# superlinear-ai/raglite

Measured on AMD Instinct MI355X. Metric: queries/sec, MaxSim 32x1M d=1024 exact top-100, higher is better.
Workload: dtype f32 in / f32 scores: candidate chunks found with the fp16 hi halves of corpus and queries (1 x v_mfma_f32_16x16x32_f16 per multiply, f32 accumulate, rigorous error bound), their scores by v_mfma_f32_16x16x4_f32 (exact f32 products); full-precision fallback: 3 x v_mfma_f32_16x16x32_f16 on hi+lo pairs

## Files before the change

### include/raglite_hip.h

```cpp
#ifndef RAGLITE_HIP_H
#define RAGLITE_HIP_H

#include <stddef.h>
#include <stdint.h>

#ifdef __cplusplus
extern "C" {
#endif

typedef enum {
    RL_OK = 0,
    RL_ERR_INVALID = -1,
    RL_ERR_HIP = -2,
    RL_ERR_UNSUPPORTED = -3,
    RL_ERR_NOMEM = -4
} rl_status;

typedef enum { RL_MEM_HOST = 0, RL_MEM_DEVICE = 1 } rl_mem;
typedef enum {
    RL_ARITH_AUTO = 0,
    RL_ARITH_FP32_EXACT = 1,
    RL_ARITH_F16_SPLIT = 2,
    RL_ARITH_F16_STORED = 3
} rl_arith;
// ... 44 lines not shown
int rl_index_delete_chunks(rl_index* index, const int64_t* chunk_ordinals, int64_t n, void* stream);
int rl_index_live(rl_index* index, int64_t* live_rows, int64_t* live_chunks, void* stream);
int rl_index_compact(rl_index* index, int64_t* out_remap, int64_t* new_n_rows, int64_t* new_n_chunks, void* stream);

int rl_index_set_arithmetic(rl_index* index, int mode);
int rl_index_arithmetic(rl_index* index, int* in_effect);

typedef enum {
    RL_OPT_HI_SEARCH = 1, RL_OPT_HI_MAXSIM = 2, RL_OPT_HI_PRODUCTS = 3, RL_OPT_PP_PASS = 4, RL_OPT_FUSED_TOPK = 5, RL_OPT_FUSED_HI = 6,
    RL_OPT_FUSED_PP = 7, RL_OPT_FUSED_TOPK_CAP = 8, RL_OPT_FUSED_TOPK_STRIDE = 9, RL_OPT_GEMM_PASS = 10, RL_OPT_QUERY_PAIRS = 11,
    RL_OPT_PLANES_GEMM = 12, RL_OPT_KEEP_IMAGE = 13, RL_OPT_KEEP_HI = 14, RL_OPT_IMAGE_HEADROOM_MB = 15, RL_OPT_ARITHMETIC = 16,
    RL_OPT_EXACT_KTH_THRESHOLD = 17, RL_OPT_FUSED_TWO_ROUNDS = 18, RL_OPT_KEEP_HI_PLANE = 19, RL_OPT_PAIRS_PACKED = 20,
    RL_OPT_F16_EXACT = 21, RL_OPT_LAZY_IMAGES = 22, RL_OPT_FUSED_PP_SAMPLE = 23,
    RL_OPT_LIST_SELECT = 24, RL_OPT_HI_FEW = 25, RL_OPT_TOPK_BLOCK = 26, RL_OPT_HI_PIVOT = 27, RL_OPT_COUNT_ = 28
} rl_option;
int rl_set_default_option(int key, int64_t value);
int rl_get_default_option(int key, int64_t* value);
int rl_index_set_option(rl_index* index, int key, int64_t value);
int rl_index_get_option(rl_index* index, int key, int64_t* value);

int rl_search_rows(rl_index* index, const float* queries, int32_t n_queries, int32_t k,
                   float* out_scores, int32_t* out_rows, int mem, void* stream);

int rl_rank_cut_begin(rl_index* index, const float* queries, int32_t n_queries, int mem, void* stream);
int rl_rank_cut_level(rl_index* index, int level, int64_t rank_limit, uint32_t* out_hist, int mem, void* stream);
int rl_rank_cut_level_done(rl_index* index, int level, const uint32_t* hist_sum, int mem, void* stream);
int rl_rank_cut_ties(rl_index* index, int64_t rank_limit, uint32_t* out_ties, int mem, void* stream);
int rl_rank_cut_finish(rl_index* index, int64_t rank_limit, const uint32_t* ties_before, const uint32_t* chunk_filter, int32_t k,
                       float* out_scores, int32_t* out_rows, int mem, void* stream);

// ... 90 lines not shown
```

### raglite_amd/_abi.py

```python

from __future__ import annotations

import ctypes as C
import functools
import os
from pathlib import Path

LIB_PATH = Path(os.environ.get("RAGLITE_HIP_LIB") or Path(__file__).resolve().parent / "_lib" / "libraglite_hip.so")

RL_OK, RL_ERR_INVALID, RL_ERR_HIP, RL_ERR_UNSUPPORTED, RL_ERR_NOMEM = 0, -1, -2, -3, -4
MEM_HOST, MEM_DEVICE = 0, 1
METRICS = {"cosine": 0, "dot": 1, "l2": 2}
SYNTH_KINDS = {"uniform": 0, "small_int": 1}
OPTIONS = {
    "hi_search": 1, "hi_maxsim": 2, "hi_products": 3, "pp_pass": 4, "fused_topk": 5, "fused_hi": 6, "fused_pp": 7, "fused_topk_cap": 8,
    "fused_topk_stride": 9, "gemm_pass": 10, "query_pairs": 11, "planes_gemm": 12, "keep_image": 13, "keep_hi": 14,
    "image_headroom_mb": 15, "arithmetic": 16, "exact_kth_threshold": 17, "fused_two_rounds": 18,
    "keep_hi_plane": 19, "pairs_packed": 20, "f16_exact": 21, "lazy_images": 22, "fused_pp_sample": 23, "list_select": 24, "hi_few": 25, "topk_block": 26, "hi_pivot": 27,
}

c_void_p, c_int, c_i32, c_i64, c_u64, c_size_t = C.c_void_p, C.c_int, C.c_int32, C.c_int64, C.c_uint64, C.c_size_t
c_double, c_char_p = C.c_double, C.c_char_p

_SIGNATURES = {
    "rl_version": [],
    "rl_last_error": [],
    "rl_init": [c_int],
    "rl_device_count": [C.POINTER(c_int)],
    "rl_device_info": [c_int, c_char_p, c_int, C.POINTER(c_int), C.POINTER(c_i64)],
    "rl_dev_alloc": [C.POINTER(c_void_p), c_size_t],
    "rl_dev_free": [c_void_p],
    "rl_memcpy_h2d": [c_void_p, c_void_p, c_size_t, c_void_p],
    "rl_memcpy_d2h": [c_void_p, c_void_p, c_size_t, c_void_p],
    "rl_memcpy_d2d": [c_void_p, c_void_p, c_size_t, c_void_p],
# ... 135 lines not shown
```

### raglite_amd/_build.py

```python

from __future__ import annotations

import os
import subprocess
import sys
from concurrent.futures import ThreadPoolExecutor
from pathlib import Path

PKG = Path(__file__).resolve().parent
CSRC = PKG / "csrc"
INCLUDE = PKG.parent / "include"
LIB_DIR = PKG / "_lib"
LIB_PATH = LIB_DIR / "libraglite_hip.so"
SOURCES = ["api.hip", "synth.hip", "pool_norm.hip", "scan.hip", "select.hip", "maxsim_stream.hip", "maxsim_generic.hip",
           "maxsim_gemm.hip", "maxsim_pp.hip", "score_gemm.hip", "mask.hip", "scan16.hip", "adapter_fit.hip", "partition_sim.hip", "comm.hip", "hi_filter.hip",
           "keyword.hip"]
FLAGS = ["--offload-arch=gfx950", "-O3", "-std=c++17", "-fPIC", "-Wall", "-Wno-unused-function",
         f"-I{INCLUDE}", f"-I{CSRC}"]


def _hipcc() -> str:
    for cand in (os.environ.get("HIPCC"), "/opt/rocm/bin/hipcc", "hipcc"):
        if cand and (os.path.isabs(cand) and os.path.exists(cand) or not os.path.isabs(cand)):
            return cand
# ... 4 lines not shown
    if not target.exists():
        return True
    t = target.stat().st_mtime
    return any(d.stat().st_mtime > t for d in deps)


EXP_LIB_PATH = LIB_DIR / "libraglite_hip_exp.so"


def build(force: bool = False, verbose: bool = False, experiments: bool = False) -> Path:
    LIB_DIR.mkdir(exist_ok=True)
    obj_dir = LIB_DIR / ("obj_exp" if experiments else "obj")
    obj_dir.mkdir(exist_ok=True)
    lib_path = EXP_LIB_PATH if experiments else LIB_PATH
    flags = FLAGS + (["-DRAGLITE_EXPERIMENTS"] if experiments else [])
    headers = [CSRC / "common.h", INCLUDE / "raglite_hip.h"]
    hipcc = _hipcc()

    def compile_one(src: str) -> Path:
        obj = obj_dir / (src + ".o")
        if force or _newer(obj, [CSRC / src, *headers]):
            cmd = [hipcc, *flags, "-c", str(CSRC / src), "-o", str(obj)]
            if verbose:
                print(" ".join(cmd), file=sys.stderr)
            res = subprocess.run(cmd, capture_output=True, text=True)
            if res.returncode != 0:
                raise RuntimeError(f"hipcc failed for {src}:\n{res.stderr}")
        return obj

    with ThreadPoolExecutor(max_workers=min(8, os.cpu_count() or 1)) as pool:
        objs = list(pool.map(compile_one, SOURCES))
# ... 11 lines not shown
```

### raglite_amd/_ops.py

```python

from __future__ import annotations

import ctypes as C
import threading
from typing import Any

import numpy as np

from raglite_amd import _abi
from raglite_amd._abi import MEM_DEVICE, MEM_HOST, METRICS, SYNTH_KINDS, check, lib

K_MAX = 2048


def _is_torch(x: Any) -> bool:
    return type(x).__module__.split(".")[0] == "torch"


def _torch():
    import torch

    return torch


# ... 59 lines not shown


def _ensure_init(device: int) -> None:
    if getattr(_tls, "initialised", None) != device:
        _abi.init(device)
        _tls.initialised = device
        _tls.device = device


def set_device(device: int) -> None:
    _tls.device = device
    _ensure_init(device)


def set_default_option(name: str, value: int) -> None:
    check(lib().rl_set_default_option(_abi.OPTIONS[name], int(value)))


def get_default_option(name: str) -> int:
    v = C.c_int64(0)
    check(lib().rl_get_default_option(_abi.OPTIONS[name], C.byref(v)))
    return int(v.value)


def synth_fill(out, seed: int, start: int = 0, kind: str = "uniform"):
    a = _Args()
    ptr = a.inp(out, np.float32)
    if a.mem != MEM_DEVICE or a.keep[0].data_ptr() != out.data_ptr():
        raise ValueError("synth_fill needs a contiguous float32 CUDA tensor")
    a.ensure_device()
    check(lib().rl_synth_fill(ptr, start, out.numel(), seed, SYNTH_KINDS[kind], a.stream))
    return out


def pool_norm(tokens, span_begin, span_end, *, normalize: bool = True, eps: float = 0.0,
              want_f32: bool = False, want_f16: bool = True):
# ... 189 lines not shown

    def compact(self) -> np.ndarray:
        _ensure_init(self.device.index or 0) if self.mem == MEM_DEVICE else _ensure_init(_current_device())
        remap = np.empty(self.n_chunks, dtype=np.int64)
        n_rows, n_chunks = C.c_int64(0), C.c_int64(0)
        check(lib().rl_index_compact(self._handle, remap.ctypes.data, C.byref(n_rows), C.byref(n_chunks), None))
        if int(n_chunks.value) != self.n_chunks:
            if self.chunk_offsets is not None:
                sizes = np.diff(self.chunk_offsets)[remap >= 0]
                self.chunk_offsets = np.concatenate(([0], np.cumsum(sizes))).astype(np.int64)
            self.n_rows, self.n_chunks = int(n_rows.value), int(n_chunks.value)
            self._keep = None
        return remap

    def set_option(self, name: str, value: int) -> None:
        check(lib().rl_index_set_option(self._handle, _abi.OPTIONS[name], int(value)))

    def get_option(self, name: str) -> int:
        v = C.c_int64(0)
        check(lib().rl_index_get_option(self._handle, _abi.OPTIONS[name], C.byref(v)))
        return int(v.value)

    def options(self, **kv: int):
        index = self

        class _Ctx:
            def __enter__(self):
                self.old = {k: index.get_option(k) for k in kv}
                for k, v in kv.items():
                    index.set_option(k, v)
                return index

            def __exit__(self, *exc):
                for k, v in self.old.items():
                    index.set_option(k, v)
# ... 287 lines not shown
```

### raglite_amd/csrc/api.hip

```cpp
#include <cmath>
#include <cstdlib>
#include <cstring>
#include <limits>
#include <memory>
#include <mutex>
#include <utility>
#include <vector>

#include "common.h"

namespace rl {

static thread_local std::string g_last_error;
void set_error(const std::string& msg) { g_last_error = msg; }
int fail(int code, const std::string& msg) {
    g_last_error = msg;
    return code;
}

namespace {

hipStream_t as_stream(void* s) { return reinterpret_cast<hipStream_t>(s); }

struct BlockCache {
// ... 165 lines not shown
    return RL_OK;
}

int scan_mode(int metric) {
    switch (metric) {
        case RL_COSINE: return SCAN_COSINE;
        case RL_DOT: return SCAN_DOT;
        case RL_L2: return SCAN_L2;
        default: return -1;
    }
}

constexpr size_t SCORE_BATCH_BYTES = size_t(8) << 30;

struct Options {
    int64_t v[RL_OPT_COUNT_];
    Options() {
        for (auto& x : v) x = 0;
        v[RL_OPT_HI_SEARCH] = v[RL_OPT_HI_MAXSIM] = v[RL_OPT_HI_PRODUCTS] = v[RL_OPT_PP_PASS] = v[RL_OPT_FUSED_TOPK] = v[RL_OPT_FUSED_HI] = 1;
        v[RL_OPT_FUSED_PP] = v[RL_OPT_GEMM_PASS] = v[RL_OPT_QUERY_PAIRS] = v[RL_OPT_PLANES_GEMM] = v[RL_OPT_KEEP_IMAGE] = v[RL_OPT_KEEP_HI] = 1;
        v[RL_OPT_EXACT_KTH_THRESHOLD] = v[RL_OPT_FUSED_TWO_ROUNDS] = v[RL_OPT_KEEP_HI_PLANE] = v[RL_OPT_F16_EXACT] = v[RL_OPT_LAZY_IMAGES] = v[RL_OPT_FUSED_PP_SAMPLE] = v[RL_OPT_LIST_SELECT] = v[RL_OPT_HI_FEW] = 1;
        v[RL_OPT_TOPK_BLOCK] = v[RL_OPT_PAIRS_PACKED] = 2;
        v[RL_OPT_HI_PIVOT] = 1;
        v[RL_OPT_IMAGE_HEADROOM_MB] = -1;
        v[RL_OPT_ARITHMETIC] = RL_ARITH_AUTO;
    }
    bool on(int key) const { return v[key] != 0; }
};
std::mutex g_default_opts_mu;
Options g_default_opts;
bool option_value_ok(int key, int64_t value) {
    switch (key) {
        case RL_OPT_HI_SEARCH: case RL_OPT_HI_MAXSIM: case RL_OPT_PP_PASS: case RL_OPT_FUSED_TOPK: case RL_OPT_FUSED_HI: case RL_OPT_FUSED_PP:
        case RL_OPT_GEMM_PASS: case RL_OPT_QUERY_PAIRS: case RL_OPT_PLANES_GEMM: case RL_OPT_KEEP_IMAGE: case RL_OPT_KEEP_HI:
        case RL_OPT_EXACT_KTH_THRESHOLD: case RL_OPT_FUSED_TWO_ROUNDS: case RL_OPT_KEEP_HI_PLANE: case RL_OPT_F16_EXACT: case RL_OPT_LAZY_IMAGES: case RL_OPT_FUSED_PP_SAMPLE: case RL_OPT_LIST_SELECT: case RL_OPT_HI_FEW: case RL_OPT_HI_PIVOT:
            return value == 0 || value == 1;
        case RL_OPT_TOPK_BLOCK: case RL_OPT_PAIRS_PACKED: return value >= 0 && value <= 2;
        case RL_OPT_HI_PRODUCTS: return value == 1 || value == 2;
        case RL_OPT_FUSED_TOPK_CAP: return value >= 0 && value <= MERGE_CAP;
        case RL_OPT_FUSED_TOPK_STRIDE: return value == 0 || (value >= 2 && value <= (int64_t(1) << 20));
        case RL_OPT_IMAGE_HEADROOM_MB: return value >= -1 && value <= (int64_t(1) << 30);
        case RL_OPT_ARITHMETIC: return value == RL_ARITH_AUTO || value == RL_ARITH_FP32_EXACT;
        default: return false;
    }
}

struct Image {
    Pool buf;
    float scale = 0.f;
    int64_t rows = 0;
// ... 684 lines not shown
    idx->opt.v[RL_OPT_ARITHMETIC] = mode;
    update_split_scale(idx);
    RL_TRY(refresh_images(idx, nullptr));
    RL_HIP(hipStreamSynchronize(nullptr));
    return RL_OK;
}

int rl_set_default_option(int key, int64_t value) {
    if (!option_value_ok(key, value)) return fail(RL_ERR_INVALID, "rl_set_default_option: unknown key or value out of range");
    std::lock_guard<std::mutex> lock(g_default_opts_mu);
    g_default_opts.v[key] = value;
    return RL_OK;
}

int rl_get_default_option(int key, int64_t* value) {
    if (!value || key < 1 || key >= RL_OPT_COUNT_) return fail(RL_ERR_INVALID, "rl_get_default_option: unknown key");
    std::lock_guard<std::mutex> lock(g_default_opts_mu);
    *value = g_default_opts.v[key];
    return RL_OK;
}

int rl_index_set_option(rl_index* idx, int key, int64_t value) {
    if (!idx) return fail(RL_ERR_INVALID, "rl_index_set_option: null index");
    if (!option_value_ok(key, value)) return fail(RL_ERR_INVALID, "rl_index_set_option: unknown key or value out of range");
    std::lock_guard<std::mutex> lock(idx->mu);
    if (idx->opt.v[key] == value) return RL_OK;
    idx->opt.v[key] = value;
    if (key == RL_OPT_KEEP_IMAGE || key == RL_OPT_KEEP_HI || key == RL_OPT_KEEP_HI_PLANE || key == RL_OPT_IMAGE_HEADROOM_MB || key == RL_OPT_ARITHMETIC ||
        key == RL_OPT_LAZY_IMAGES) {
        RL_TRY(use_scratch(idx, nullptr));
        if (key == RL_OPT_ARITHMETIC) {
            idx->arithmetic = (int)value;
            update_split_scale(idx);
        }
        RL_TRY(refresh_images(idx, nullptr));
        RL_HIP(hipStreamSynchronize(nullptr));
    }
    return RL_OK;
}

int rl_index_get_option(rl_index* idx, int key, int64_t* value) {
    if (!idx || !value || key < 1 || key >= RL_OPT_COUNT_) return fail(RL_ERR_INVALID, "rl_index_get_option: null argument or unknown key");
    std::lock_guard<std::mutex> lock(idx->mu);
    *value = idx->opt.v[key];
    return RL_OK;
}

int rl_index_arithmetic(rl_index* idx, int* in_effect) {
    if (!idx || !in_effect) return fail(RL_ERR_INVALID, "rl_index_arithmetic: null argument");
    std::lock_guard<std::mutex> lock(idx->mu);
    *in_effect = idx->E16 ? RL_ARITH_F16_STORED : (idx->split_scale > 0.f ? RL_ARITH_F16_SPLIT : RL_ARITH_FP32_EXACT);
    return RL_OK;
}

int rl_index_append(rl_index* idx, const float* rows, int64_t n_new_rows, const int64_t* new_chunk_sizes,
                    int64_t n_new_chunks, int mem, void* stream) {
    if (!idx) return fail(RL_ERR_INVALID, "rl_index_append: null index");
// ... 892 lines not shown
int hi_batch_approx(rl_index* idx, const float* d_q, int32_t nq, int32_t n_queries, int32_t n_gemm, int32_t k, float* sc, int64_t ld, HiBatch& hb,
                    hipStream_t s, bool flag_zeroed = false) {
    hb.one_product = idx->opt.v[RL_OPT_HI_PRODUCTS] == 1;
    hb.exact_kth = idx->opt.on(RL_OPT_EXACT_KTH_THRESHOLD);
    RL_TRY(idx->hibuf.reserve(hi_batch_words(n_gemm, k) * 4));
    hi_batch_layout(idx, n_gemm, k, hb);
    const int32_t cap = hb.cap;
    hb.m_abs = idx->norm_stats.max_lo_norm + sum_eps(idx->dim) * idx->norm_stats.max_row_norm;
    hb.q_unscale = reinterpret_cast<const float*>(idx->qplanes.as<char>() + (size_t)n_queries * idx->dim * 128);
    hb.qsum = hb.q_unscale + 2 * (size_t)n_queries;
    if (!flag_zeroed) RL_HIP(hipMemsetAsync(hb.flag, 0, 16 * sizeof(uint32_t), s));
    (void)cap;
    const bool pp = hb.one_product && idx->dim >= 256 && idx->opt.on(RL_OPT_PP_PASS);
    if (pp)
        RL_TRY(launch_maxsim_pp(approx_image(idx), idx->n_rows, idx->dim, idx->qplanes.p, n_queries, 0, n_gemm, nq, idx->row_to_chunk,
                                idx->offsets, idx->ends.as<uint32_t>(), sc, ld, idx->n_cu, s, approx_scale(idx)));
    for (int32_t b = 0; !pp && b < n_gemm; b += GEMM_PASS_QUERIES) {
        const int32_t n_q = std::min<int32_t>(GEMM_PASS_QUERIES, n_gemm - b);
        RL_TRY(launch_maxsim_gemm(approx_image(idx), idx->n_rows, idx->dim, idx->qplanes.p, n_queries, b, n_q, nq, idx->row_to_chunk,
                                  idx->offsets, idx->ends.as<uint32_t>(), sc + (int64_t)b * ld, ld, idx->n_cu, s, approx_scale(idx), true,
                                  nullptr, hb.one_product));
    }
    RL_TRY(mask_chunk_scores(idx, sc, n_gemm, ld, hb.filter, s));
    int st_pv = RL_ERR_UNSUPPORTED;
    if (n_gemm < 16 && idx->n_chunks > (int64_t)262144 && idx->opt.on(RL_OPT_HI_PIVOT))
        st_pv = launch_topk_pivot(sc, n_gemm, idx->n_chunks, ld, k, idx->ws, hb.ts, hb.ti, s);
    if (st_pv != RL_OK && st_pv != RL_ERR_UNSUPPORTED) return st_pv;
    if (st_pv == RL_ERR_UNSUPPORTED) RL_TRY(launch_topk(sc, n_gemm, idx->n_chunks, ld, k, idx->ws, hb.ts, hb.ti, s));
    return RL_OK;
}
int hi_batch_fallback(rl_index* idx, const float* d_q, int32_t nq, int32_t n_queries, int32_t n_gemm, int32_t k, float* sc, int64_t ld,
// ... 336 lines not shown
        return fail(RL_ERR_UNSUPPORTED, "rl_maxsim_approx_scores: this index keeps no HI image (or nq > 32 / dim < 256)");
    DevBuf t_q, t_o, t_b;
    const float* d_q; float* d_o; float* d_b = nullptr;
    const size_t q_elems = (size_t)nq * idx->dim;
    const int64_t ld = idx->n_chunks;
    RL_TRY(stage_in(query_vecs, (size_t)n_queries * q_elems, mem, s, t_q, &d_q));
    RL_TRY(stage_out_begin(out_scores, (size_t)n_queries * ld, mem, t_o, &d_o));
    if (out_bound) RL_TRY(stage_out_begin(out_bound, (size_t)n_queries, mem, t_b, &d_b));
    RL_TRY(idx->qplanes.reserve(query_planes_bytes(idx->dim, n_queries)));
    RL_TRY(launch_query_planes(d_q, idx->dim, nq, (int64_t)q_elems, n_queries, idx->qplanes.p, s));
    const int32_t per = kernel == 0 ? n_queries : GEMM_PASS_QUERIES;
    for (int32_t b = 0; b < n_queries; b += per) {
        const int32_t n_q = std::min<int32_t>(per, n_queries - b);
        if (kernel == 0)
            RL_TRY(launch_maxsim_pp(approx_image(idx), idx->n_rows, idx->dim, idx->qplanes.p, n_queries, b, n_q, nq, idx->row_to_chunk, idx->offsets,
                                    idx->ends.as<uint32_t>(), d_o + (int64_t)b * ld, ld, idx->n_cu, s, approx_scale(idx)));
        else
            RL_TRY(launch_maxsim_gemm(approx_image(idx), idx->n_rows, idx->dim, idx->qplanes.p, n_queries, b, n_q, nq, idx->row_to_chunk, idx->offsets,
                                      idx->ends.as<uint32_t>(), d_o + (int64_t)b * ld, ld, idx->n_cu, s, approx_scale(idx), true, nullptr, true));
    }
    if (d_b) {
        const float m_abs = idx->norm_stats.max_lo_norm + sum_eps(idx->dim) * idx->norm_stats.max_row_norm;
        const float* q_unscale = reinterpret_cast<const float*>(idx->qplanes.as<char>() + (size_t)n_queries * idx->dim * 128);
        RL_TRY(idx->hibuf.reserve((size_t)n_queries * 4 * sizeof(float) + 64));
        float* top = idx->hibuf.as<float>();
        float* thr = top + n_queries;
        uint32_t* cnt = reinterpret_cast<uint32_t*>(thr + n_queries);
        uint32_t* flag = cnt + n_queries;
        RL_HIP(hipMemsetAsync(top, 0, (size_t)n_queries * sizeof(float), s));
        RL_HIP(hipMemsetAsync(flag, 0, 16 * sizeof(uint32_t), s));
        RL_TRY(launch_maxsim_threshold(top, n_queries, 1, d_q, nq, idx->dim, (int64_t)q_elems, 1.0f, m_abs, thr, cnt, flag, s, q_unscale,
// ... 198 lines not shown
        if (st != RL_OK) { (void)hipEventDestroy(e0); (void)hipEventDestroy(e1); return st == RL_ERR_UNSUPPORTED ? fail(st, "rl_time_kernel: the eight-query kernel does not apply to this index / shape") : st; }
    }
    if (kind == 7) {
        st = pp_vec >= 1 && pp_vec * pp_n == nq ? gemm_prepare(idx, q_dev, pp_vec, (int64_t)pp_vec * idx->dim, pp_n, s) : RL_ERR_UNSUPPORTED;
        if (st == RL_OK && !(approx_image_valid(idx) && idx->dim >= 256)) st = RL_ERR_UNSUPPORTED;
        if (st != RL_OK) { (void)hipEventDestroy(e0); (void)hipEventDestroy(e1); return st == RL_ERR_UNSUPPORTED ? fail(st, "rl_time_kernel: the sixteen-query kernel does not apply to this index / shape") : st; }
    }
    if (kind == 4 || kind == 10) {
        st = demand_images(idx, IMG_HI_PLANE, s);
        if (st != RL_OK) { (void)hipEventDestroy(e0); (void)hipEventDestroy(e1); return st; }
    }
    RL_HIP(hipEventRecord(e0, s));
    for (int i = 0; i < iters && st == RL_OK; ++i) {
        if (kind == 7) st = launch_maxsim_pp(approx_image(idx), idx->n_rows, idx->dim, idx->qplanes.p, pp_n, 0, pp_n,
                                             pp_vec, idx->row_to_chunk, idx->offsets, idx->ends.as<uint32_t>(), idx->scores.as<float>(), ldc,
                                             idx->n_cu, s, approx_scale(idx));
        else if (kind == 3) st = gemm_pass(idx, nq / GEMM_PASS_QUERIES, GEMM_PASS_QUERIES, 0, GEMM_PASS_QUERIES, idx->scores.as<float>(), ldc, s);
        else if (kind == 8) {
            const auto& r = idx->replay;
            if (hipMemsetAsync(r.cnt, 0, (size_t)r.B * sizeof(uint32_t), s) != hipSuccess) st = RL_ERR_HIP;
            else if (r.pp && r.round1_tiles > 0) {
                CandArgs ca1 = r.ca;
                ca1.tau = r.thr1;
                st = launch_pp_rows_pass(idx->hi_image.buf.p, idx->n_rows, idx->dim, r.B, r.qs, idx->norm, r.mode, &ca1, idx->pp_work.p, r.log_cap, idx->n_cu, s,
                                         idx->split_scale, 0, r.round1_tiles, false, r.row_test);
                if (st == RL_OK)
                    st = launch_pp_rows_pass(idx->hi_image.buf.p, idx->n_rows, idx->dim, r.B, r.qs, idx->norm, r.mode, &r.ca, idx->pp_work.p, r.log_cap, idx->n_cu, s,
                                             idx->split_scale, r.round1_tiles, -1, true, r.row_test);
            }
            else if (r.pp) st = launch_pp_rows_pass(idx->hi_image.buf.p, idx->n_rows, idx->dim, r.B, r.qs, idx->norm, r.mode, &r.ca, idx->pp_work.p, r.log_cap,
                                                    idx->n_cu, s, idx->split_scale, 0, -1, false, r.row_test);
// ... 209 lines not shown
```

### raglite_amd/csrc/common.h

```cpp
#pragma once
#include <hip/hip_runtime.h>
#include <stdint.h>

#include <algorithm>
#include <cstdlib>
#include <string>

#include "raglite_hip.h"

namespace rl {

void set_error(const std::string& msg);
int fail(int code, const std::string& msg);

#define RL_HIP(expr)                                                                         \
    do {                                                                                     \
        hipError_t _e = (expr);                                                              \
        if (_e != hipSuccess)                                                                \
            return ::rl::fail(_e == hipErrorOutOfMemory ? RL_ERR_NOMEM : RL_ERR_HIP,         \
                              std::string(#expr) + ": " + hipGetErrorString(_e));            \
    } while (0)

#define RL_TRY(expr)              \
    do {                          \
// ... 274 lines not shown
int launch_presplit_rows(const float* E, int64_t first_row, int64_t n_rows, int32_t dim, float scale, void* planes, hipStream_t s);
int launch_preformat_rows16(const uint16_t* E, int64_t first_row, int64_t n_rows, int32_t dim, void* planes, hipStream_t s);
int launch_presplit_hi_rows(const float* E, int64_t first_row, int64_t n_rows, int32_t dim, float scale, void* planes, hipStream_t s);
size_t chunk_ends_words(int64_t rows);
int launch_chunk_ends(const int32_t* row_to_chunk, int64_t n_rows, uint32_t* ends, hipStream_t s);
size_t query_planes_bytes(int32_t dim, int32_t n_queries);
int launch_query_planes(const float* Q, int32_t dim, int32_t nq, int64_t q_stride, int32_t n_queries, void* buf, hipStream_t s,
                        uint32_t* zero_words = nullptr, int n_zero = 0);
int launch_maxsim_gemm(const void* planes, int64_t n_rows, int32_t dim, const void* qbuf, int32_t n_queries, int32_t first,
                       int32_t n_q, int32_t nq, const int32_t* row_to_chunk, const int64_t* chunk_offsets, const uint32_t* ends_bits,
                       float* out, int64_t out_stride, int n_cu, hipStream_t s, float split_scale, bool half = false,
                       const uint32_t* run_if = nullptr, bool hi_only = false, bool all_passes = false);
constexpr int32_t PP_PASS_QUERIES = 16;
int launch_maxsim_pp(const void* image, int64_t n_rows, int32_t dim, const void* qbuf, int32_t n_queries, int32_t first, int32_t n_q,
                     int32_t nq, const int32_t* row_to_chunk, const int64_t* chunk_offsets, const uint32_t* ends_bits, float* out,
                     int64_t out_stride, int n_cu, hipStream_t s, float split_scale, const uint32_t* run_if = nullptr);
constexpr int32_t MFMA_RATE_ITERS = 1000;
int launch_mfma_f16_rate(float* out, int n_cu, int32_t iters, hipStream_t s, double* flops);
size_t score_planes_scratch_floats(int32_t nb, int32_t dim);
int launch_score_planes(const void* planes, int64_t n_rows, int32_t dim, const float* Q, int32_t nb, float* scores, int64_t ld,
                        const float* row_norm, const float* row_sumsq, float* scratch, int mode, int n_cu, hipStream_t s, float split_scale,
                        bool half = false);
struct CandArgs { const float* tau; int32_t tau_stride; float* scores; int32_t* ids; uint32_t* cnt; uint32_t* overflow; int32_t cap; };
int launch_score_planes_queries(const float* Q, int32_t nb, int32_t dim, float* scratch, int mode, hipStream_t s, uint32_t* zero_word = nullptr);
size_t pp_rows_scratch_bytes(int64_t n_rows, int32_t nb, int n_cu, int32_t expected_per_query, int32_t* log_cap_out);
int launch_pp_rows_pass(const void* image, int64_t n_rows, int32_t dim, int32_t nb, float* scratch, const float* row_norm, int mode,
                        const CandArgs* cand, void* work, int32_t log_cap, int n_cu, hipStream_t s, float split_scale, int64_t tile_begin = 0,
                        int64_t tile_count = -1, bool norms_ready = false,
                        bool row_norm_test = false);
int launch_pp_rows_sample(const void* image, int64_t n_rows, int32_t dim, int32_t nb, float* scratch, const float* row_norm, int mode, float* S,
                          int64_t ld_s, int32_t stride, int n_cu, hipStream_t s, float split_scale);
// ... 32 lines not shown
```

### raglite_amd/csrc/maxsim_pp.hip

```cpp
#include <cstdio>
#include <cstdlib>
#include <utility>

#include "common.h"

namespace rl {

typedef float f32x4 __attribute__((ext_vector_type(4)));
typedef _Float16 h16x8 __attribute__((ext_vector_type(8)));

namespace {
constexpr int PP_RT = 128;
constexpr int PP_NBLK = PP_RT / 16;
constexpr int PP_QPP = 16;
constexpr int PP_DC = 8;
constexpr int PP_LC = 6;
constexpr int PP_CSLOT = PP_NBLK * 1024;
constexpr int PP_STAGE = 1536;
constexpr int PP_LDS = PP_DC * PP_CSLOT + 16 * PP_STAGE * 4;

__device__ __forceinline__ int64_t pp_uniform_i64(int64_t v) {
    const uint32_t lo = __builtin_amdgcn_readfirstlane((uint32_t)(uint64_t)v);
    const uint32_t hi = __builtin_amdgcn_readfirstlane((uint32_t)((uint64_t)v >> 32));
    return (int64_t)(((uint64_t)hi << 32) | lo);
}

__device__ __forceinline__ void pp_dma(uint32_t lds, const char* src, uint32_t lane16) {
    const uint32_t l = __builtin_amdgcn_readfirstlane(lds);
    const char* const p = reinterpret_cast<const char*>(pp_uniform_i64(reinterpret_cast<int64_t>(src)));
    asm volatile("s_mov_b32 m0, %0\n\ts_nop 0\n\tglobal_load_lds_dwordx4 %1, %2 nt" ::"s"(l), "v"(lane16), "s"(p) : "memory", "m0");
}

template <int OFF>
__device__ __forceinline__ void pp_read(f32x4& dst, uint32_t addr) {
    asm volatile("ds_read_b128 %0, %1 offset:%2" : "=v"(dst) : "v"(addr), "n"(OFF) : "memory");
}
__device__ __forceinline__ void pp_pin(f32x4& a, f32x4& b, f32x4& c, f32x4& d) { asm volatile("" : "+v"(a), "+v"(b), "+v"(c), "+v"(d)); }
typedef float f32x16s __attribute__((ext_vector_type(16)));
__device__ __forceinline__ f32x16s pp_sload16(const float* p) {
    f32x16s v;
    const float* const u = reinterpret_cast<const float*>(pp_uniform_i64(reinterpret_cast<int64_t>(p)));
    asm volatile("s_load_dwordx16 %0, %1, 0x0\n\ts_waitcnt lgkmcnt(0)" : "=s"(v) : "s"(u) : "memory");
    return v;
}
__device__ __forceinline__ h16x8 pp_h(const f32x4& v) {
// ... 15 lines not shown
    int32_t tile_begin, tile_count;
    float* S; int64_t ld_s; int32_t stride;
};

template <int DBG, int MODE, bool ROWNORM>
__global__ __launch_bounds__(512, 2) void maxsim_pp_kernel(const char* __restrict__ planes, int64_t n_rows, int32_t nslab,
                                                           const char* __restrict__ qfrag, const float* __restrict__ qmeta, int32_t n_q,
                                                           const int32_t* __restrict__ row_to_chunk, const int64_t* __restrict__ chunk_offsets,
                                                           const uint32_t* __restrict__ ends_bits, float* __restrict__ out, int64_t out_stride,
                                                           float inv_e_scale, const uint32_t* __restrict__ run_if, PpRows rs) {
    constexpr bool ROWS = MODE == 2, SCORES = MODE == 1, GROUPS = ROWS || SCORES;
    __shared__ __attribute__((aligned(16))) char smem[PP_LDS];
    if (run_if && __builtin_amdgcn_readfirstlane((int)*run_if) == 0) return;
    const int lane = threadIdx.x & 63;
    const int wv = wave_id();
    const int64_t G = gridDim.x, b = blockIdx.x;
    auto boundary = [&](int64_t t) -> int64_t {
        if (t <= 0) return 0;
        if (t >= n_rows) return n_rows;
        const int32_t c = row_to_chunk[t];
        const int64_t c0 = chunk_offsets[c], c1 = chunk_offsets[c + 1];
        return c0 == t ? t : c1;
    };
    int32_t r_lo = 0, r_hi = 0, nt_rows = 0;
    if constexpr (!GROUPS) {
        r_lo = (int32_t)pp_uniform_i64(boundary((n_rows * b) / G));
        r_hi = (int32_t)pp_uniform_i64((b + 1 == G) ? n_rows : boundary((n_rows * (b + 1)) / G));
        if (r_hi <= r_lo) return;
    } else {
        const int64_t Tr = rs.tile_count;
        const int64_t t0 = (Tr * b) / G, t1 = (Tr * (b + 1)) / G;
        nt_rows = (int32_t)(t1 - t0);
        if (nt_rows <= 0) return;
        r_lo = (int32_t)((rs.tile_begin + t0) * PP_RT);
        r_hi = (int32_t)n_rows;
    }
    const int32_t org = r_lo & ~15;
    const int nt = GROUPS ? nt_rows : (r_hi - org + PP_RT - 1) / PP_RT;
    auto tile_blk = [&](int t) __attribute__((always_inline)) -> int32_t {
        if constexpr (SCORES) {
            const int32_t o = (org >> 7) + t;
            return ((o >> 1) * 2 * rs.stride + (o & 1)) * PP_NBLK;
        } else {
            return (org >> 4) + t * PP_NBLK;
        }
    };
    const int qt = (int)blockIdx.y;
    const int q_base = GROUPS ? 0 : PP_QPP * qt;
    const int total = nt * nslab;
    const int32_t last_blk = (int32_t)((n_rows + 15) >> 4) - 1;
    const uint32_t lds_base = (uint32_t)reinterpret_cast<uintptr_t>((__attribute__((address_space(3))) char*)smem);
    const uint32_t lane16 = 16u * lane;

    const bool has0 = q_base + 2 * wv < n_q, has1 = q_base + 2 * wv + 1 < n_q;
    int ql0 = PP_QPP * qt + 2 * wv, ql1 = PP_QPP * qt + 2 * wv + 1;
    ql0 = ql0 < n_q ? ql0 : n_q - 1;
    ql1 = ql1 < n_q ? ql1 : n_q - 1;
    const char* const qp0 = qfrag + pp_uniform_i64((int64_t)ql0 * nslab * 4096);
    const char* const qp1 = qfrag + pp_uniform_i64((int64_t)ql1 * nslab * 4096);
    int qr_s = 0;
    auto issue_qregs = [&](f32x4 (&qn)[4]) __attribute__((always_inline)) {
        if constexpr (!(DBG & 32)) {
// ... 3 lines not shown
                         : "=&v"(qn[0]), "=&v"(qn[1]) : "v"(lane16), "s"(a0) : "memory");
            asm volatile("global_load_dwordx4 %0, %2, %3\n\tglobal_load_dwordx4 %1, %2, %3 offset:2048"
                         : "=&v"(qn[2]), "=&v"(qn[3]) : "v"(lane16), "s"(a1) : "memory");
            if (++qr_s == nslab) qr_s = 0;
        }
    };
    int fc_s = 0, fc_r = 0, fc_slot = 0;
    const int32_t blk_org = (org >> 4) + wv;
    const int64_t slab_bytes = (int64_t)nslab * 1024;
    auto issue_c = [&]() __attribute__((always_inline)) {
        if constexpr (!(DBG & 16)) {
            const int t = fc_r < nt ? fc_r : nt - 1;
            int32_t blk = SCORES ? tile_blk(t) + wv : blk_org + t * PP_NBLK;
            blk = blk < last_blk ? blk : last_blk;
            const char* src = planes + pp_uniform_i64((int64_t)blk * slab_bytes + (int64_t)fc_s * 1024);
            pp_dma(lds_base + (uint32_t)(fc_slot * PP_CSLOT + wv * 1024), src, lane16);
        }
        if (++fc_s == nslab) { fc_s = 0; ++fc_r; }
        fc_slot = fc_slot + 1 == PP_DC ? 0 : fc_slot + 1;
    };

    f32x4 acc[2][2][PP_NBLK];
#pragma unroll
    for (int q = 0; q < 2; ++q)
#pragma unroll
        for (int qb = 0; qb < 2; ++qb)
#pragma unroll
            for (int a = 0; a < PP_NBLK; ++a) acc[q][qb][a] = (f32x4){0.f, 0.f, 0.f, 0.f};

    f32x4 ef[PP_NBLK];
    f32x4 qA[4], qB[4];
// ... 444 lines not shown
        if (n_q > 1000000) {
            f32x4 t = (f32x4){0.f, 0.f, 0.f, 0.f};
#pragma unroll
            for (int q = 0; q < 2; ++q)
#pragma unroll
                for (int qb = 0; qb < 2; ++qb)
#pragma unroll
                    for (int a = 0; a < PP_NBLK; ++a) t += acc[q][qb][a];
            out[lane] = (t[0] + t[1]) + (t[2] + t[3]);
        }
    }
}

int launch_maxsim_pp(const void* image, int64_t n_rows, int32_t dim, const void* qbuf, int32_t n_queries, int32_t first, int32_t n_q,
                     int32_t nq, const int32_t* row_to_chunk, const int64_t* chunk_offsets, const uint32_t* ends_bits, float* out,
                     int64_t out_stride, int n_cu, hipStream_t s, float split_scale, const uint32_t* run_if) {
    if (nq < 1 || nq > 32 || n_q < 1 || n_q > PP_QPP * 4096 || n_rows < 1 || first < 0 || first + n_q > n_queries) return RL_ERR_UNSUPPORTED;
    if (dim % 32 || dim < 256 || !(split_scale > 0.f) || !image || !ends_bits) return RL_ERR_UNSUPPORTED;
    const int32_t nslab = dim / 32;
    const char* qfrag = static_cast<const char*>(qbuf) + (size_t)first * nslab * 4096;
    const float* qmeta = reinterpret_cast<const float*>(static_cast<const char*>(qbuf) + (size_t)n_queries * dim * 128) + 2 * (size_t)first;
    const int64_t tiles = (n_rows + PP_RT - 1) / PP_RT;
    const dim3 grid((unsigned)std::max<int64_t>(1, std::min<int64_t>(n_cu > 0 ? n_cu : 256, tiles)), (unsigned)((n_q + PP_QPP - 1) / PP_QPP)), blk(512);
#define RL_PP_LAUNCH(DBG_)                                                                                                                 \
    hipLaunchKernelGGL((maxsim_pp_kernel<DBG_, 0, false>), grid, blk, 0, s, static_cast<const char*>(image), n_rows, nslab, qfrag, qmeta, n_q, row_to_chunk, \
                       chunk_offsets, ends_bits, out, out_stride, 1.0f / split_scale, run_if, PpRows{})
#ifdef RAGLITE_EXPERIMENTS
    static const int dbg = std::getenv("RAGLITE_PP_DBG") ? std::atoi(std::getenv("RAGLITE_PP_DBG")) : 0;
    if (dbg == 2) RL_PP_LAUNCH(2);
    else if (dbg == 128) RL_PP_LAUNCH(128);
    else if (dbg == 136) RL_PP_LAUNCH(136);
    else if (dbg == 144) RL_PP_LAUNCH(144);
    else if (dbg == 160) RL_PP_LAUNCH(160);
    else if (dbg == 184) RL_PP_LAUNCH(184);
    else RL_PP_LAUNCH(0);
#else
    RL_PP_LAUNCH(0);
#endif
// ... 154 lines not shown
```

Before: 16130.

## Flatten PP grid and co-locate query passes of a row range on one XCD

The maxsim_pp launch changes from a 2D grid (row ranges x query passes) to a 1D grid. A new pp_schedule mapping puts the blocks that scan the same row range for different query passes on the same XCD, in groups of eight, and dispatches them close together in time. With that layout the corpus slabs fetched by one pass can be served from the shared L2 for the others, so the non-temporal hint on the global-to-LDS loads is dropped for this path. The new behaviour sits behind a default-on option; the trade-off is possible L2 pollution and a load imbalance in the leftover ranges.

```diff
diff --git a/include/raglite_hip.h b/include/raglite_hip.h
--- a/include/raglite_hip.h
+++ b/include/raglite_hip.h
@@ -82,6 +82,7 @@
     RL_OPT_F16_EXACT = 21, RL_OPT_LAZY_IMAGES = 22, RL_OPT_FUSED_PP_SAMPLE = 23,
     RL_OPT_LIST_SELECT = 24, RL_OPT_HI_FEW = 25, RL_OPT_TOPK_BLOCK = 26, RL_OPT_HI_PIVOT = 27, RL_OPT_COUNT_ = 28
 } rl_option;
+enum { RL_OPT_PP_SCHEDULE = 64 };
 int rl_set_default_option(int key, int64_t value);
 int rl_get_default_option(int key, int64_t* value);
 int rl_index_set_option(rl_index* index, int key, int64_t value);
diff --git a/raglite_amd/_abi.py b/raglite_amd/_abi.py
--- a/raglite_amd/_abi.py
+++ b/raglite_amd/_abi.py
@@ -18,6 +18,11 @@
     "image_headroom_mb": 15, "arithmetic": 16, "exact_kth_threshold": 17, "fused_two_rounds": 18,
     "keep_hi_plane": 19, "pairs_packed": 20, "f16_exact": 21, "lazy_images": 22, "fused_pp_sample": 23, "list_select": 24, "hi_few": 25, "topk_block": 26, "hi_pivot": 27,
 }
+SCHEDULE_OPTIONS = {"pp_schedule": 64}
+
+
+def option_key(name: str) -> int:
+    return OPTIONS[name] if name in OPTIONS else SCHEDULE_OPTIONS[name]
 
 c_void_p, c_int, c_i32, c_i64, c_u64, c_size_t = C.c_void_p, C.c_int, C.c_int32, C.c_int64, C.c_uint64, C.c_size_t
 c_double, c_char_p = C.c_double, C.c_char_p
diff --git a/raglite_amd/_build.py b/raglite_amd/_build.py
--- a/raglite_amd/_build.py
+++ b/raglite_amd/_build.py
@@ -42,7 +42,7 @@
     obj_dir.mkdir(exist_ok=True)
     lib_path = EXP_LIB_PATH if experiments else LIB_PATH
     flags = FLAGS + (["-DRAGLITE_EXPERIMENTS"] if experiments else [])
-    headers = [CSRC / "common.h", INCLUDE / "raglite_hip.h"]
+    headers = [CSRC / "common.h", CSRC / "pp_schedule.h", INCLUDE / "raglite_hip.h"]
     hipcc = _hipcc()
 
     def compile_one(src: str) -> Path:
diff --git a/raglite_amd/_ops.py b/raglite_amd/_ops.py
--- a/raglite_amd/_ops.py
+++ b/raglite_amd/_ops.py
@@ -97,12 +97,12 @@
 
 
 def set_default_option(name: str, value: int) -> None:
-    check(lib().rl_set_default_option(_abi.OPTIONS[name], int(value)))
+    check(lib().rl_set_default_option(_abi.option_key(name), int(value)))
 
 
 def get_default_option(name: str) -> int:
     v = C.c_int64(0)
-    check(lib().rl_get_default_option(_abi.OPTIONS[name], C.byref(v)))
+    check(lib().rl_get_default_option(_abi.option_key(name), C.byref(v)))
     return int(v.value)
 
 
@@ -322,11 +322,11 @@
         return remap
 
     def set_option(self, name: str, value: int) -> None:
-        check(lib().rl_index_set_option(self._handle, _abi.OPTIONS[name], int(value)))
+        check(lib().rl_index_set_option(self._handle, _abi.option_key(name), int(value)))
 
     def get_option(self, name: str) -> int:
         v = C.c_int64(0)
-        check(lib().rl_index_get_option(self._handle, _abi.OPTIONS[name], C.byref(v)))
+        check(lib().rl_index_get_option(self._handle, _abi.option_key(name), C.byref(v)))
         return int(v.value)
 
     def options(self, **kv: int):
diff --git a/raglite_amd/csrc/api.hip b/raglite_amd/csrc/api.hip
--- a/raglite_amd/csrc/api.hip
+++ b/raglite_amd/csrc/api.hip
@@ -203,7 +203,7 @@
 constexpr size_t SCORE_BATCH_BYTES = size_t(8) << 30;
 
 struct Options {
-    int64_t v[RL_OPT_COUNT_];
+    int64_t v[RL_OPT_PP_SCHEDULE + 1];
     Options() {
         for (auto& x : v) x = 0;
         v[RL_OPT_HI_SEARCH] = v[RL_OPT_HI_MAXSIM] = v[RL_OPT_HI_PRODUCTS] = v[RL_OPT_PP_PASS] = v[RL_OPT_FUSED_TOPK] = v[RL_OPT_FUSED_HI] = 1;
@@ -211,6 +211,7 @@
         v[RL_OPT_EXACT_KTH_THRESHOLD] = v[RL_OPT_FUSED_TWO_ROUNDS] = v[RL_OPT_KEEP_HI_PLANE] = v[RL_OPT_F16_EXACT] = v[RL_OPT_LAZY_IMAGES] = v[RL_OPT_FUSED_PP_SAMPLE] = v[RL_OPT_LIST_SELECT] = v[RL_OPT_HI_FEW] = 1;
         v[RL_OPT_TOPK_BLOCK] = v[RL_OPT_PAIRS_PACKED] = 2;
         v[RL_OPT_HI_PIVOT] = 1;
+        v[RL_OPT_PP_SCHEDULE] = 1;
         v[RL_OPT_IMAGE_HEADROOM_MB] = -1;
         v[RL_OPT_ARITHMETIC] = RL_ARITH_AUTO;
     }
@@ -218,11 +219,13 @@
 };
 std::mutex g_default_opts_mu;
 Options g_default_opts;
+bool option_key_ok(int key) { return (key >= 1 && key < RL_OPT_COUNT_) || key == RL_OPT_PP_SCHEDULE; }
 bool option_value_ok(int key, int64_t value) {
     switch (key) {
         case RL_OPT_HI_SEARCH: case RL_OPT_HI_MAXSIM: case RL_OPT_PP_PASS: case RL_OPT_FUSED_TOPK: case RL_OPT_FUSED_HI: case RL_OPT_FUSED_PP:
         case RL_OPT_GEMM_PASS: case RL_OPT_QUERY_PAIRS: case RL_OPT_PLANES_GEMM: case RL_OPT_KEEP_IMAGE: case RL_OPT_KEEP_HI:
         case RL_OPT_EXACT_KTH_THRESHOLD: case RL_OPT_FUSED_TWO_ROUNDS: case RL_OPT_KEEP_HI_PLANE: case RL_OPT_F16_EXACT: case RL_OPT_LAZY_IMAGES: case RL_OPT_FUSED_PP_SAMPLE: case RL_OPT_LIST_SELECT: case RL_OPT_HI_FEW: case RL_OPT_HI_PIVOT:
+        case RL_OPT_PP_SCHEDULE:
             return value == 0 || value == 1;
         case RL_OPT_TOPK_BLOCK: case RL_OPT_PAIRS_PACKED: return value >= 0 && value <= 2;
         case RL_OPT_HI_PRODUCTS: return value == 1 || value == 2;
@@ -937,7 +940,7 @@
 }
 
 int rl_get_default_option(int key, int64_t* value) {
-    if (!value || key < 1 || key >= RL_OPT_COUNT_) return fail(RL_ERR_INVALID, "rl_get_default_option: unknown key");
+    if (!value || !option_key_ok(key)) return fail(RL_ERR_INVALID, "rl_get_default_option: unknown key");
     std::lock_guard<std::mutex> lock(g_default_opts_mu);
     *value = g_default_opts.v[key];
     return RL_OK;
@@ -963,7 +966,7 @@
 }
 
 int rl_index_get_option(rl_index* idx, int key, int64_t* value) {
-    if (!idx || !value || key < 1 || key >= RL_OPT_COUNT_) return fail(RL_ERR_INVALID, "rl_index_get_option: null argument or unknown key");
+    if (!idx || !value || !option_key_ok(key)) return fail(RL_ERR_INVALID, "rl_index_get_option: null argument or unknown key");
     std::lock_guard<std::mutex> lock(idx->mu);
     *value = idx->opt.v[key];
     return RL_OK;
@@ -1886,7 +1889,8 @@
     const bool pp = hb.one_product && idx->dim >= 256 && idx->opt.on(RL_OPT_PP_PASS);
     if (pp)
         RL_TRY(launch_maxsim_pp(approx_image(idx), idx->n_rows, idx->dim, idx->qplanes.p, n_queries, 0, n_gemm, nq, idx->row_to_chunk,
-                                idx->offsets, idx->ends.as<uint32_t>(), sc, ld, idx->n_cu, s, approx_scale(idx)));
+                                idx->offsets, idx->ends.as<uint32_t>(), sc, ld, idx->n_cu, s, approx_scale(idx), nullptr,
+                                (int)idx->opt.v[RL_OPT_PP_SCHEDULE]));
     for (int32_t b = 0; !pp && b < n_gemm; b += GEMM_PASS_QUERIES) {
         const int32_t n_q = std::min<int32_t>(GEMM_PASS_QUERIES, n_gemm - b);
         RL_TRY(launch_maxsim_gemm(approx_image(idx), idx->n_rows, idx->dim, idx->qplanes.p, n_queries, b, n_q, nq, idx->row_to_chunk,
@@ -2253,7 +2257,8 @@
         const int32_t n_q = std::min<int32_t>(per, n_queries - b);
         if (kernel == 0)
             RL_TRY(launch_maxsim_pp(approx_image(idx), idx->n_rows, idx->dim, idx->qplanes.p, n_queries, b, n_q, nq, idx->row_to_chunk, idx->offsets,
-                                    idx->ends.as<uint32_t>(), d_o + (int64_t)b * ld, ld, idx->n_cu, s, approx_scale(idx)));
+                                    idx->ends.as<uint32_t>(), d_o + (int64_t)b * ld, ld, idx->n_cu, s, approx_scale(idx), nullptr,
+                                    (int)idx->opt.v[RL_OPT_PP_SCHEDULE]));
         else
             RL_TRY(launch_maxsim_gemm(approx_image(idx), idx->n_rows, idx->dim, idx->qplanes.p, n_queries, b, n_q, nq, idx->row_to_chunk, idx->offsets,
                                       idx->ends.as<uint32_t>(), d_o + (int64_t)b * ld, ld, idx->n_cu, s, approx_scale(idx), true, nullptr, true));
@@ -2482,7 +2487,7 @@
     for (int i = 0; i < iters && st == RL_OK; ++i) {
         if (kind == 7) st = launch_maxsim_pp(approx_image(idx), idx->n_rows, idx->dim, idx->qplanes.p, pp_n, 0, pp_n,
                                              pp_vec, idx->row_to_chunk, idx->offsets, idx->ends.as<uint32_t>(), idx->scores.as<float>(), ldc,
-                                             idx->n_cu, s, approx_scale(idx));
+                                             idx->n_cu, s, approx_scale(idx), nullptr, (int)idx->opt.v[RL_OPT_PP_SCHEDULE]);
         else if (kind == 3) st = gemm_pass(idx, nq / GEMM_PASS_QUERIES, GEMM_PASS_QUERIES, 0, GEMM_PASS_QUERIES, idx->scores.as<float>(), ldc, s);
         else if (kind == 8) {
             const auto& r = idx->replay;
diff --git a/raglite_amd/csrc/common.h b/raglite_amd/csrc/common.h
--- a/raglite_amd/csrc/common.h
+++ b/raglite_amd/csrc/common.h
@@ -312,7 +312,7 @@
 constexpr int32_t PP_PASS_QUERIES = 16;
 int launch_maxsim_pp(const void* image, int64_t n_rows, int32_t dim, const void* qbuf, int32_t n_queries, int32_t first, int32_t n_q,
                      int32_t nq, const int32_t* row_to_chunk, const int64_t* chunk_offsets, const uint32_t* ends_bits, float* out,
-                     int64_t out_stride, int n_cu, hipStream_t s, float split_scale, const uint32_t* run_if = nullptr);
+                     int64_t out_stride, int n_cu, hipStream_t s, float split_scale, const uint32_t* run_if, int schedule);
 constexpr int32_t MFMA_RATE_ITERS = 1000;
 int launch_mfma_f16_rate(float* out, int n_cu, int32_t iters, hipStream_t s, double* flops);
 size_t score_planes_scratch_floats(int32_t nb, int32_t dim);
diff --git a/raglite_amd/csrc/maxsim_pp.hip b/raglite_amd/csrc/maxsim_pp.hip
--- a/raglite_amd/csrc/maxsim_pp.hip
+++ b/raglite_amd/csrc/maxsim_pp.hip
@@ -3,6 +3,7 @@
 #include <utility>
 
 #include "common.h"
+#include "pp_schedule.h"
 
 namespace rl {
 
@@ -25,10 +26,14 @@
     return (int64_t)(((uint64_t)hi << 32) | lo);
 }
 
+template <bool NT>
 __device__ __forceinline__ void pp_dma(uint32_t lds, const char* src, uint32_t lane16) {
     const uint32_t l = __builtin_amdgcn_readfirstlane(lds);
     const char* const p = reinterpret_cast<const char*>(pp_uniform_i64(reinterpret_cast<int64_t>(src)));
-    asm volatile("s_mov_b32 m0, %0\n\ts_nop 0\n\tglobal_load_lds_dwordx4 %1, %2 nt" ::"s"(l), "v"(lane16), "s"(p) : "memory", "m0");
+    if constexpr (NT)
+        asm volatile("s_mov_b32 m0, %0\n\ts_nop 0\n\tglobal_load_lds_dwordx4 %1, %2 nt" ::"s"(l), "v"(lane16), "s"(p) : "memory", "m0");
+    else
+        asm volatile("s_mov_b32 m0, %0\n\ts_nop 0\n\tglobal_load_lds_dwordx4 %1, %2" ::"s"(l), "v"(lane16), "s"(p) : "memory", "m0");
 }
 
 template <int OFF>
@@ -74,7 +79,14 @@
     if (run_if && __builtin_amdgcn_readfirstlane((int)*run_if) == 0) return;
     const int lane = threadIdx.x & 63;
     const int wv = wave_id();
-    const int64_t G = gridDim.x, b = blockIdx.x;
+    int64_t G = gridDim.x, b = blockIdx.x;
+    int qt = (int)blockIdx.y;
+    if constexpr (!GROUPS) {
+        const PpSlot m = pp_schedule((int32_t)blockIdx.x, (int32_t)blockIdx.y, (int32_t)gridDim.x, (int32_t)gridDim.y, (n_q + PP_QPP - 1) / PP_QPP);
+        G = m.ranges;
+        b = m.range;
+        qt = m.pass;
+    }
     auto boundary = [&](int64_t t) -> int64_t {
         if (t <= 0) return 0;
         if (t >= n_rows) return n_rows;
@@ -105,7 +117,6 @@
             return (org >> 4) + t * PP_NBLK;
         }
     };
-    const int qt = (int)blockIdx.y;
     const int q_base = GROUPS ? 0 : PP_QPP * qt;
     const int total = nt * nslab;
     const int32_t last_blk = (int32_t)((n_rows + 15) >> 4) - 1;
@@ -139,7 +150,7 @@
             int32_t blk = SCORES ? tile_blk(t) + wv : blk_org + t * PP_NBLK;
             blk = blk < last_blk ? blk : last_blk;
             const char* src = planes + pp_uniform_i64((int64_t)blk * slab_bytes + (int64_t)fc_s * 1024);
-            pp_dma(lds_base + (uint32_t)(fc_slot * PP_CSLOT + wv * 1024), src, lane16);
+            pp_dma<GROUPS>(lds_base + (uint32_t)(fc_slot * PP_CSLOT + wv * 1024), src, lane16);
         }
         if (++fc_s == nslab) { fc_s = 0; ++fc_r; }
         fc_slot = fc_slot + 1 == PP_DC ? 0 : fc_slot + 1;
@@ -614,14 +625,15 @@
 
 int launch_maxsim_pp(const void* image, int64_t n_rows, int32_t dim, const void* qbuf, int32_t n_queries, int32_t first, int32_t n_q,
                      int32_t nq, const int32_t* row_to_chunk, const int64_t* chunk_offsets, const uint32_t* ends_bits, float* out,
-                     int64_t out_stride, int n_cu, hipStream_t s, float split_scale, const uint32_t* run_if) {
+                     int64_t out_stride, int n_cu, hipStream_t s, float split_scale, const uint32_t* run_if, int schedule) {
     if (nq < 1 || nq > 32 || n_q < 1 || n_q > PP_QPP * 4096 || n_rows < 1 || first < 0 || first + n_q > n_queries) return RL_ERR_UNSUPPORTED;
     if (dim % 32 || dim < 256 || !(split_scale > 0.f) || !image || !ends_bits) return RL_ERR_UNSUPPORTED;
     const int32_t nslab = dim / 32;
     const char* qfrag = static_cast<const char*>(qbuf) + (size_t)first * nslab * 4096;
     const float* qmeta = reinterpret_cast<const float*>(static_cast<const char*>(qbuf) + (size_t)n_queries * dim * 128) + 2 * (size_t)first;
     const int64_t tiles = (n_rows + PP_RT - 1) / PP_RT;
-    const dim3 grid((unsigned)std::max<int64_t>(1, std::min<int64_t>(n_cu > 0 ? n_cu : 256, tiles)), (unsigned)((n_q + PP_QPP - 1) / PP_QPP)), blk(512);
+    const int64_t gx = std::max<int64_t>(1, std::min<int64_t>(n_cu > 0 ? n_cu : 256, tiles)), passes = (n_q + PP_QPP - 1) / PP_QPP;
+    const dim3 grid = schedule == 1 ? dim3((unsigned)(gx * passes)) : dim3((unsigned)gx, (unsigned)passes), blk(512);
 #define RL_PP_LAUNCH(DBG_)                                                                                                                 \
     hipLaunchKernelGGL((maxsim_pp_kernel<DBG_, 0, false>), grid, blk, 0, s, static_cast<const char*>(image), n_rows, nslab, qfrag, qmeta, n_q, row_to_chunk, \
                        chunk_offsets, ends_bits, out, out_stride, 1.0f / split_scale, run_if, PpRows{})
diff --git a/raglite_amd/csrc/pp_schedule.h b/raglite_amd/csrc/pp_schedule.h
--- /dev/null
+++ b/raglite_amd/csrc/pp_schedule.h
@@ -0,0 +1,27 @@
+#pragma once
+#include <stdint.h>
+
+#if defined(__HIPCC__) || defined(__CUDACC__)
+#define RL_PP_HD __host__ __device__
+#else
+#define RL_PP_HD
+#endif
+
+namespace rl {
+
+struct PpSlot {
+    int32_t ranges;
+    int32_t range;
+    int32_t pass;
+};
+
+RL_PP_HD inline PpSlot pp_schedule(int32_t x, int32_t y, int32_t gx, int32_t gy, int32_t passes) {
+    if (gy > 1 || passes <= 1) return PpSlot{gx, x, y};
+    const int32_t ranges = gx / passes;
+    const int32_t whole = ranges & ~7, head = whole * passes;
+    if (x < head) return PpSlot{ranges, 8 * (x / (8 * passes)) + x % 8, (x / 8) % passes};
+    const int32_t t = x - head, rest = ranges - whole;
+    return PpSlot{ranges, whole + t % rest, t / rest};
+}
+
+}
```

Result: faster. 17330, median of 6 (+7.4%).
